# liruiluo/VLA-Adapter

Hardware: AMD Instinct MI355X
Metric: fine-tune samples/sec (224px img + 32-tok prompt), adapter-only, fwd+bwd+AdamW (higher is better)
Workload: dtype bf16

## Files before the change

include/vla_native.h:

```cpp
#ifndef VLA_NATIVE_H
#define VLA_NATIVE_H
#ifdef __cplusplus
extern "C" {
#endif

#define VLA_ERR_ARG (-1)
#define VLA_ERR_LAUNCH (-2)
#define VLA_ERR_UNSUPPORTED (-3)

#define VLA_ABI_VERSION 8
int vla_version(void);
int vla_desc_size(int which);
const char* vla_last_error(void);

enum { VLA_ACT_NONE = 0, VLA_ACT_GELU = 1, VLA_ACT_RELU = 2, VLA_ACT_GELU_TANH = 3, VLA_ACT_SWIGLU = 4, VLA_ACT_SWIGLU_BWD = 5 };

typedef struct vla_gemm_desc {
  const void* A;
  const void* B;
  void* C;
  const void* bias;
  const void* R;
  void* C2;
  int M, N, K, lda, ldb, ldc, ldr, ldc2;
// ... 49 lines not shown
int vla_layernorm_fwd_q8(void* stream, const void* x, const void* w, const void* b, void* y, float* stats, void* q8, float* qscale, int rows,
                         int cols, int ldx, int ldy, int ldq, float eps);

int vla_gemm_bf16_nt(void* stream, const vla_gemm_desc* desc );

int vla_transpose_bf16(void* stream, const void* in, void* out, int rows, int cols, int ldi, int ldo, int batch,
                       long long s_in, long long s_out);

int vla_layernorm_fwd(void* stream, const void* x, const void* w, const void* b, void* y, float* stats, int rows,
                      int cols, int ldx, int ldy, float eps);
int vla_layernorm_bwd(void* stream, const void* dy, const void* x, const void* w, const float* stats, void* dx,
                      float* dw, float* db, int rows, int cols, int ldx, int lddy, int lddx);
int vla_rmsnorm_fwd(void* stream, const void* x, const void* w, void* y, float* rstd, int rows, int cols, float eps);
int vla_rmsnorm_bwd(void* stream, const void* dy, const void* x, const void* w, const float* rstd, const void* dres,
                    void* dx, int rows, int cols, int x_group, int x_group_rows, int x_row0);

int vla_rmsnorm_dw(void* stream, const void* dy, const void* x, const float* rstd, float* dw, int rows, int cols);

typedef struct vla_attn_desc {
  const void* q; const void* k; const void* v;
  void* o;
  float* lse;
  const unsigned char* kmask;
  long long q_sb, k_sb, v_sb, o_sb;
  int q_ss, k_ss, v_ss, o_ss;
  int B, Sq, Sk, Hq, Hkv, dh, causal;
  float scale;
  const void* dout; void* dq; void* dk; void* dv; float* delta;
  long long do_sb, dq_sb, dk_sb, dv_sb; int do_ss, dq_ss, dk_ss, dv_ss;
  const float* rope_cos; const float* rope_sin;
// ... 117 lines not shown
```

vla_adapter_amd/csrc/gemm.hip:

```cpp
#include <algorithm>
#include "common.h"
#include "gemm_params.h"
#include "../../include/vla_native.h"

namespace {

constexpr int BK = 64;
constexpr int EPI_PAD = 16;


__device__ __forceinline__ float apply_act(float v, int act) {
  switch (act) {
    case VLA_ACT_GELU: return rbf(gelu_erf(v));
    case VLA_ACT_RELU: return fmaxf(v, 0.f);
    case VLA_ACT_GELU_TANH: return rbf(gelu_tanh(v));
    default: return v;
  }
}

typedef int v8i_f8 __attribute__((ext_vector_type(8)));
__device__ __forceinline__ v8i_f8 cat8(bf16x8 lo, bf16x8 hi) {
  typedef float f32x8 __attribute__((ext_vector_type(8)));
  const f32x4 l = __builtin_bit_cast(f32x4, lo), h = __builtin_bit_cast(f32x4, hi);
  return __builtin_bit_cast(v8i_f8, f32x8{l[0], l[1], l[2], l[3], h[0], h[1], h[2], h[3]});
// ... 668 lines not shown
  if (d->fp8)
    VLA_REQUIRE(d->fp8 == 1 && d->a_scale && d->b_scale && d->K % 128 == 0 && d->lda % 16 == 0 && d->ldb % 16 == 0 && d->batch == 1 &&
                    d->split_k <= 1 && d->rope_mode != 2 && d->a_group == 0 && (d->act != VLA_ACT_SWIGLU_BWD || d->K2 > 0),
                "gemm: fp8 needs scales, K % 128 == 0, 16-B rows, batch 1, no split-K / interleaved RoPE / row groups on A (SwiGLU backward: with a K extension only)");
  VLA_REQUIRE(((uintptr_t)d->A & 15) == 0 && ((uintptr_t)d->B & 15) == 0, "gemm: A/B must be 16-B aligned");
  VLA_REQUIRE(d->sA % 8 == 0 && d->sB % 8 == 0, "gemm: batch strides of A/B must keep 16-B alignment");
  if (d->act == VLA_ACT_SWIGLU_BWD) {
    VLA_REQUIRE(d->C && d->R && !d->bias && d->rope_mode == 0 && d->N % 64 == 0 && d->ldc % 8 == 0 && d->ldr % 4 == 0 &&
                    ((uintptr_t)d->R & 7) == 0 && d->c_group == 0 && d->res_mod == 0,
                "gemm: swiglu_bwd needs C = dGU [M, 2N] (ldc%8), R = GU [M, 2N] (interleaved), N%64 == 0");
  } else if (d->act == VLA_ACT_SWIGLU) {
    VLA_REQUIRE(d->C2 && d->N % 32 == 0 && d->ldc2 % 4 == 0 && ((uintptr_t)d->C2 & 7) == 0 && d->sC2 % 4 == 0,
                "gemm: swiglu needs C2, N%32==0, ldc2%4==0");
    VLA_REQUIRE(!d->R, "gemm: swiglu epilogue takes no residual");
  } else {
    VLA_REQUIRE(d->C, "gemm: null C");
  }
  if (d->C) VLA_REQUIRE(((uintptr_t)d->C & 15) == 0 || (d->ldc % 8) != 0, "gemm: C must be 16-B aligned");
  if (d->C && d->ldc % 8 == 0) VLA_REQUIRE(d->sC % 8 == 0, "gemm: sC must keep 16-B alignment");
  if (d->R && d->ldc % 8 == 0 && d->ldr % 8 == 0 && d->act != VLA_ACT_SWIGLU_BWD)
    VLA_REQUIRE(((uintptr_t)d->R & 15) == 0 && d->sR % 8 == 0, "gemm: R must be 16-B aligned");
  VLA_REQUIRE(d->a_group >= 0 && d->c_group >= 0 && d->a_group_stride % 8 == 0 &&
                  (d->c_group == 0 || d->ldc % 8 != 0 || d->c_group_stride % 8 == 0),
              "gemm: row-group strides must keep 16-B alignment");
  const bool split_k = d->split_k > 1;
  VLA_REQUIRE(d->bias_post_round == 0 || (d->bias_post_round == 1 && d->bias && d->rope_mode != 1 && !split_k && d->act == VLA_ACT_NONE),
              "gemm: bias_post_round needs a bias and a plain epilogue (no rotate_half rope / split-K / activation)");
  if (split_k) {
    VLA_REQUIRE(d->ws && d->batch == 1 && d->rope_mode == 0 && d->c_group == 0 && d->r_group == 0 &&
                    d->res_mod == 0 && d->c_live_mod == 0 && d->C &&
                    (d->act == VLA_ACT_NONE || d->act == VLA_ACT_GELU || d->act == VLA_ACT_RELU || d->act == VLA_ACT_GELU_TANH),
                "gemm: split_k needs an fp32 workspace [split_k, M, N], batch 1 and a plain epilogue");
    VLA_REQUIRE(d->N % 4 == 0 && ((uintptr_t)d->ws & 15) == 0, "gemm: split_k needs N % 4 == 0 and a 16-B aligned workspace");
  }
  VLA_REQUIRE(d->c_live_mod >= 0 && d->c_live_from >= 0 && (d->c_live_mod == 0 || d->c_live_from < d->c_live_mod),
              "gemm: c_live_from must lie inside c_live_mod");
  VLA_REQUIRE(d->r_group >= 0 && d->r_group_stride % 8 == 0 && (d->r_group == 0 || d->res_mod == 0),
              "gemm: r_group stride must keep 16-B alignment; r_group and res_mod are exclusive");
  if (d->K2 != 0)
    VLA_REQUIRE(d->K2 > 0 && d->K2 % BK == 0 && d->A2 && d->B2 && d->lda2 % 8 == 0 && d->ldb2 % 8 == 0 && (((uintptr_t)d->A2 | (uintptr_t)d->B2) & 15) == 0 &&
                    d->batch == 1 && !split_k && d->rope_mode != 2,
                "gemm: the K extension needs A2 / B2 (bf16, 16-B aligned rows, K2 % 64 == 0), batch 1, no split-K / interleaved RoPE");
  if (d->rope_mode != 0) {
    VLA_REQUIRE(d->rope_mode == 1 || d->rope_mode == 2, "gemm: rope_mode 0/1/2");
    VLA_REQUIRE(d->rope_cos && d->rope_sin && d->rope_T > 0 && d->rope_dh > 0 && d->rope_dh % 4 == 0 && d->rope_cols % 64 == 0 &&
                    (((uintptr_t)d->rope_cos | (uintptr_t)d->rope_sin) & 15) == 0 && d->act != VLA_ACT_SWIGLU,
                "gemm: bad rope arguments");
// ... 39 lines not shown
  else if (pl.kernel == VLA_KERNEL_NT_256)
    rc = vla_gemm256_launch(p, d->act == VLA_ACT_SWIGLU ? 1 : d->act == VLA_ACT_SWIGLU_BWD ? 2 : 0, d->batch, ov.grid_set ? ov.grid : ncu, st);
  else if (d->K2 > 0 && d->fp8)
    rc = rope == 3 ? launch_nt<3, true, true>(pl.kernel, p, nb, st) : rope == 1 ? launch_nt<1, true, true>(pl.kernel, p, nb, st)
                                                                                : launch_nt<0, true, true>(pl.kernel, p, nb, st);
  else if (d->K2 > 0)
    rc = rope == 3 ? launch_nt<3, false, true>(pl.kernel, p, nb, st) : rope == 1 ? launch_nt<1, false, true>(pl.kernel, p, nb, st)
                                                                                 : launch_nt<0, false, true>(pl.kernel, p, nb, st);
  else if (d->fp8) rc = rope == 1 ? launch_nt<1, true>(pl.kernel, p, nb, st) : launch_nt<0, true>(pl.kernel, p, nb, st);
  else if (rope == 3) rc = launch_nt<3>(pl.kernel, p, nb, st);
  else if (rope == 2) rc = launch_nt<2>(pl.kernel, p, nb, st);
  else if (rope == 1) rc = launch_nt<1>(pl.kernel, p, nb, st);
  else rc = launch_nt<0>(pl.kernel, p, nb, st);
  if (rc) return rc;
  VLA_CHECK_LAUNCH("gemm_bf16_nt");
  if (pl.split > 1) return splitk_finalize(d, pl.split, st);
  return VLA_OK;
}
```

vla_adapter_amd/csrc/norm.hip:

```cpp
#include "common.h"
#include "../../include/vla_native.h"

namespace {

template <int NCH>
__device__ __forceinline__ void load_row(const bf16_t* x, int cols, int lane, uint4 (&v)[NCH]) {
#pragma unroll
  for (int c = 0; c < NCH; ++c) {
    const int e = (c * 64 + lane) * 8;
    v[c] = (e < cols) ? *reinterpret_cast<const uint4*>(x + e) : uint4{0, 0, 0, 0};
  }
}
__device__ __forceinline__ void unpack8(const uint4& u, float (&f)[8]) {
  const unsigned w[4] = {u.x, u.y, u.z, u.w};
#pragma unroll
  for (int k = 0; k < 4; ++k) {
    f[2 * k] = __uint_as_float(w[k] << 16);
    f[2 * k + 1] = __uint_as_float(w[k] & 0xffff0000u);
  }
}
__device__ __forceinline__ uint4 pack8(const float (&f)[8]) {
  return uint4{pack2(f[0], f[1]), pack2(f[2], f[3]), pack2(f[4], f[5]), pack2(f[6], f[7])};
}

// ... 193 lines not shown
  for (int c = 0; c < NCH; ++c) {
    const int e = (c * 64 + lane) * 8;
    if (e >= cols) continue;
    float f[8], fw[8], o[8];
    unpack8(v[c], f);
    unpack8(vw[c], fw);
#pragma unroll
    for (int k = 0; k < 8; ++k) o[k] = fw[k] * rbf(f[k] * rstd);
    v[c] = pack8(o);
    if (y) *reinterpret_cast<uint4*>(y + (long long)row * cols + e) = v[c];
  }
  if (q8) quant_row_q8<NCH>(v, cols, lane, q8 + (long long)row * ldq, qscale + row);
}

template <int NCH>
__global__ __launch_bounds__(256) void rmsnorm_bwd_kernel(const bf16_t* __restrict__ dy, const bf16_t* __restrict__ x,
                                                          const bf16_t* __restrict__ w, const float* __restrict__ rstd_in,
                                                          const bf16_t* __restrict__ dres, bf16_t* __restrict__ dx,
                                                          int rows, int cols, int xg, int xgr, int xr0) {
  const int lane = threadIdx.x & 63;
  const int row = blockIdx.x * 4 + (threadIdx.x >> 6);
  if (row >= rows) return;
  const long long xrow = xg > 0 ? (long long)(row / xg) * xgr + xr0 + (row % xg) : row;
  uint4 vx[NCH], vd[NCH], vw[NCH], vr[NCH];
  load_row<NCH>(x + xrow * cols, cols, lane, vx);
  load_row<NCH>(dy + (long long)row * cols, cols, lane, vd);
  load_row<NCH>(w, cols, lane, vw);
  if (dres) load_row<NCH>(dres + (long long)row * cols, cols, lane, vr);
  const float rstd = rstd_in[xrow];
  float s = 0.f;
#pragma unroll
  for (int c = 0; c < NCH; ++c) {
    const int e = (c * 64 + lane) * 8;
    if (e >= cols) continue;
    float fx[8], fd[8], fw[8];
    unpack8(vx[c], fx);
    unpack8(vd[c], fd);
    unpack8(vw[c], fw);
#pragma unroll
    for (int k = 0; k < 8; ++k) s += fd[k] * fw[k] * fx[k] * rstd;
  }
  s = wave_sum(s) / cols;
#pragma unroll
  for (int c = 0; c < NCH; ++c) {
    const int e = (c * 64 + lane) * 8;
    if (e >= cols) continue;
    float fx[8], fd[8], fw[8], o[8];
    unpack8(vx[c], fx);
    unpack8(vd[c], fd);
    unpack8(vw[c], fw);
    float fr[8] = {0, 0, 0, 0, 0, 0, 0, 0};
    if (dres) unpack8(vr[c], fr);
#pragma unroll
    for (int k = 0; k < 8; ++k) o[k] = fr[k] + rstd * (fd[k] * fw[k] - fx[k] * rstd * s);
    *reinterpret_cast<uint4*>(dx + (long long)row * cols + e) = pack8(o);
  }
}

inline int nch_for(int cols) { return (cols + 511) / 512; }

#define DISPATCH_NCH(n, CALL)                    \
  if (n <= 1) { CALL(1); }                       \
  else if (n <= 2) { CALL(2); }                  \
  else if (n <= 3) { CALL(3); }                  \
  else if (n <= 4) { CALL(4); }                  \
  else if (n <= 8) { CALL(8); }                  \
  else if (n <= 16) { CALL(16); }                \
  else { CALL(24); }

// ... 72 lines not shown
extern "C" int vla_rmsnorm_fwd_q8(void* stream, const void* x, const void* w, void* y, float* rstd, void* q8, float* qscale, int rows, int cols,
                                  int ldq, float eps) {
  VLA_REQUIRE(x && w && q8 && qscale && rows > 0 && cols > 0, "rmsnorm_fwd_q8: null/empty");
  VLA_REQUIRE(cols % 8 == 0 && cols <= 12288 && ldq % 16 == 0 && ldq >= cols, "rmsnorm_fwd_q8: cols%8==0, cols<=12288, ldq%16");
  VLA_REQUIRE((((uintptr_t)x | (uintptr_t)y | (uintptr_t)w | (uintptr_t)q8) & 15) == 0, "rmsnorm_fwd_q8: 16-B alignment");
  const int n = nch_for(cols);
  dim3 grid((rows + 3) / 4);
#define CALL(N) hipLaunchKernelGGL(rmsnorm_fwd_kernel<N>, grid, dim3(256), 0, (hipStream_t)stream, (const bf16_t*)x, (const bf16_t*)w, (bf16_t*)y, \
                                   rstd, rows, cols, eps, (unsigned char*)q8, qscale, ldq)
  DISPATCH_NCH(n, CALL)
#undef CALL
  VLA_CHECK_LAUNCH("rmsnorm_fwd_q8");
  return VLA_OK;
}

extern "C" int vla_rmsnorm_bwd(void* stream, const void* dy, const void* x, const void* w, const float* rstd,
                               const void* dres, void* dx, int rows, int cols, int x_group, int x_group_rows, int x_row0) {
  VLA_REQUIRE(dy && x && w && rstd && dx && rows > 0 && cols > 0, "rmsnorm_bwd: null/empty");
  VLA_REQUIRE(x_group >= 0 && (x_group == 0 || (x_row0 >= 0 && x_row0 + x_group <= x_group_rows)), "rmsnorm_bwd: bad row window");
  VLA_REQUIRE(cols % 8 == 0 && cols <= 12288, "rmsnorm_bwd: cols%8==0");
  const int n = nch_for(cols);
  dim3 grid((rows + 3) / 4);
#define CALL(N) hipLaunchKernelGGL(rmsnorm_bwd_kernel<N>, grid, dim3(256), 0, (hipStream_t)stream, (const bf16_t*)dy, \
                                   (const bf16_t*)x, (const bf16_t*)w, rstd, (const bf16_t*)dres, (bf16_t*)dx, rows, cols, \
                                   x_group, x_group_rows, x_row0)
  DISPATCH_NCH(n, CALL)
#undef CALL
  VLA_CHECK_LAUNCH("rmsnorm_bwd");
  return VLA_OK;
}


template <int LPR>
__global__ __launch_bounds__(CR_THREADS) void rmsnorm_dw_kernel(const bf16_t* __restrict__ dy, const bf16_t* __restrict__ x,
                                                                const float* __restrict__ rstd, float* __restrict__ dw, int rows, int cols) {
  __shared__ float sm[CR_THREADS / 64][64];
  const int c = CR<LPR>::col();
  float a[8] = {0, 0, 0, 0, 0, 0, 0, 0};
  if (c < cols)
    for (int r = CR<LPR>::row0(); r < rows; r += CR<LPR>::GROUPS) {
      float fd[8], fx[8];
      unpack8(*reinterpret_cast<const uint4*>(dy + (long long)r * cols + c), fd);
      unpack8(*reinterpret_cast<const uint4*>(x + (long long)r * cols + c), fx);
#pragma unroll
// ... 25 lines not shown
```

vla_adapter_amd/engine.py:

```python
from __future__ import annotations

import math
import os
from dataclasses import dataclass, field
from typing import Dict, List, Optional, Tuple

import torch

from . import ops, schedule
from .ops import ACT_GELU, ACT_GELU_TANH, ACT_NONE, ACT_RELU, ACT_SWIGLU, BF16
from .schedule import Segment, capture_graph, chunks, turnaround_chunks

NUM_TOKENS = 64
IGNORE_INDEX = -100


def rup(n: int, m: int) -> int:
    return (n + m - 1) // m * m


def copy_flat(dst: torch.Tensor, src: torch.Tensor):
    n = src.numel()
    ops.copy2d(src, dst, 1, n, n, n)

# ... 155 lines not shown
        q, s_ = self._qscratch(x.shape[0], x.shape[1], "n")
        ops.rmsnorm_fwd_q8(x, w, eps, q, s_, rstd=rstd, y=out if self.keep_norm_out else None)
        return self._hand_over(out, q, s_)

    def _lin(self, key, x, W, bias=None, **kw):
        wq = self.Q.get(key)
        if wq is not None:
            xq, xs = self._quant(x, "f")
            return ops.gemm_nt(xq, wq[0], bias=bias, fp8=(xs, wq[1]), **kw)
        return ops.gemm_nt(x, W, bias=bias, **kw)

    def _lin_bwd(self, key, dy, x, WT, out=None, swiglu_gu=None, **kw):
        if swiglu_gu is not None:
            return ops.gemm_swiglu_bwd(dy, WT, swiglu_gu, out=out, **kw)
        return ops.gemm_nt(dy, WT, out=out)


class ViT:

    def __init__(self, cfg: ViTCfg, sd: Dict[str, torch.Tensor], device, j: int = 0):
        self.cfg, self.key = cfg, f"vit{j}."
        self.lin = Linear(device)
        d, P = cfg.d, cfg.patch
        g = lambda k: sd[k].to(device=device, dtype=BF16).contiguous()
        self.kpe = rup(3 * P * P, 64)
        wpe = torch.zeros(d, self.kpe, device=device, dtype=BF16)
        wpe[:, :3 * P * P] = g("patch_embed.proj.weight").reshape(d, -1)
        self.wpe, self.bpe = wpe, g("patch_embed.proj.bias")
        self.pos = g("pos_embed").reshape(-1, d)
        assert self.pos.shape[0] == cfg.n_patches, "pos_embed covers patches only (no_embed_class / no cls token)"
# ... 194 lines not shown

    def fwd_final(self):
        n, D = self.cfg.n_layers, self.cfg.d
        ops.rmsnorm_fwd(self.HS[n + 1].view(-1, D), self.norm, self.cfg.eps, out=self.HS[n].view(-1, D), rstd=self.RF)

    def enable_fp8(self):
        for i, L in enumerate(self.layers):
            self.lin.Q[f"llm.{i}.qkv"] = ops.quant_fp8_rows(L["wqkv"])
            self.lin.Q[f"llm.{i}.gu"] = ops.quant_fp8_rows(L["wgu"])
        self.lin.fp8 = True

    def backward(self, dHS: torch.Tensor, B: int, S: int, row0: int = 0, n_run: Optional[int] = None) -> torch.Tensor:
        n_run = self.cfg.n_layers if n_run is None else n_run
        self.bwd_begin(dHS, row0, n_run)
        for i in range(n_run - 1, -1, -1):
            self.bwd_layer(i, dHS)
        return self.bwd_result()

    def bwd_begin(self, dHS: torch.Tensor, row0: Optional[int] = 0, n_run: Optional[int] = None, lin: Optional[Linear] = None):
        n, S, D = self.cfg.n_layers, self.S, self.cfg.d
        self._n_run = n if n_run is None else n_run
        self._blin = lin = self.lin if lin is None else lin
        if row0 is None:
            self.r0, self.Rl, self._win = 0, S, None
        else:
            assert 0 <= row0 < S and row0 % 32 == 0, "live-row window must start on a multiple of 32"
            assert row0 >= self.gu_row0, "the forward dropped backward-only rows this window needs"
            self.r0, self.Rl = row0, S - row0
            self._win = (self.Rl, S, row0)
        Mr = self.B * self.Rl
        assert tuple(dHS.shape[1:]) == (self.B, self.Rl, D)
        d = (self.G_res[self._n_run - 1] if self.per_layer else self.d_a)[:Mr]
        if self._n_run == n:
            self._d = ops.rmsnorm_bwd(dHS[n].view(Mr, D), self.HS[n + 1].view(-1, D), self.norm, self.RF, out=d, x_rows=self._win)
            if lin.trains_vectors:
                ops.rmsnorm_dw(dHS[n].view(Mr, D), self.HS[n + 1].view(-1, D), self.RF, lin.A("llm.norm"))
        else:
            self._d = ops.copy2d(dHS[self._n_run].view(Mr, D), d, Mr, D, D, D)

    def bwd_layer(self, i: int, dHS: torch.Tensor):
        c, B, S, r0, R, lin = self.cfg, self.B, self.S, self.r0, self.Rl, self._blin
        M, D, H, KV, dh, I = B * S, c.d, c.heads, c.kv_heads, c.dh, c.inter
        Mr, tv, win = B * R, lin.trains_vectors, self._win
        L, k, d = self.layers[i], f"llm.{i}.", self._d
        _, n2, h = self._keeps(i)
        if self.per_layer:
            d1_out, d_out = self.G_d1[i], (self.G_res[i - 1] if i > 0 else self.d_last)[:Mr]
            d_gu, d_qkv = self.G_gu[i][:Mr], self.G_qkv[i][:Mr]
        else:
            d1_out, d_out, d_gu, d_qkv = self.d_b[:Mr], d, self.d_gu[:Mr], self.d_qkv[:Mr]
        if i < self._n_run - 1:
            ops.add_(d, dHS[i + 1].view(Mr, D))
        tap = lin.taps.get(("llm", i)) if lin.taps is not None else None
        if tap is not None:
            tap["d_out"] = d.clone()
        d_gu = lin._lin_bwd(k + "down", d, h, L["wdT"], out=d_gu, swiglu_gu=self.GU[i][r0:], **({"gu_group": (R, S * 2 * I)} if win else {}))
        d_n = lin._lin_bwd(k + "gu", d_gu, n2, L["wguT"], out=self.G_n2[i] if tv else self.d_n[:Mr])
        if tv:
            lin._defer(lambda dy=d_n, x=self.X1[i], r=self.R2[i], acc=lin.A(k + "n2"): ops.rmsnorm_dw(dy, x, r, acc))
        d1 = ops.rmsnorm_bwd(d_n, self.X1[i], L["n2"], self.R2[i], dres=d, out=d1_out, x_rows=win)
        dao = lin._lin_bwd(k + "o", d1, self.AO[i], L["woT"], out=self.d_n[:Mr])
        q, kk, v = self._attn_views(self.QKV[i].view(B, S, -1))
        dq, dk, dv = self._attn_views(d_qkv.view(B, R, -1))
        ops.attn_bwd(dao.view(B, R, -1), q[:, r0:], kk, v, self.AO[i].view(B, S, -1)[:, r0:], self.LSE[i], H, KV, dh, True,
                     self.kmask, dq=dq, dk=dk, dv=dv, rope=(self.cos, self.sin) if dh in (64, 128) else None, row0=r0)
        if dh not in (64, 128):
            cs, sn = self.cos[r0:], self.sin[r0:]
            ops.rope_half_(d_qkv[:, :H * dh], cs, sn, R, H, dh, sign=-1)
            ops.rope_half_(d_qkv[:, H * dh:(H + KV) * dh], cs, sn, R, KV, dh, sign=-1)
        d_n = lin._lin_bwd(k + "qkv", d_qkv, self._keeps(i)[0], L["wqkvT"], out=self.G_n1[i] if tv else self.d_n[:Mr])
        if tv:
            lin._defer(lambda dy=d_qkv, acc=lin.A(k + "bqkv"): ops.colsum_(dy, acc))
            lin._defer(lambda dy=d_n, x=self.HS[i].view(M, D), r=self.R1[i], acc=lin.A(k + "n1"): ops.rmsnorm_dw(dy, x, r, acc))
        self._d = ops.rmsnorm_bwd(d_n, self.HS[i].view(M, D), L["n1"], self.R1[i], dres=d1, out=d_out, x_rows=win)
        if tap is not None:
            tap["d_in"] = self._d.clone()

    def bwd_result(self) -> torch.Tensor:
        return self._d.view(self.B, self.Rl, self.cfg.d)


class FlatParams:

    def __init__(self, spec: List[Tuple[str, Tuple[int, ...]]], device):
        self.offsets, off = {}, 0
        for name, shape in spec:
            n = math.prod(shape)
            self.offsets[name] = (off, shape)
            off += rup(n, 8)
        self.numel = off
        self.data = torch.zeros(off, device=device, dtype=BF16)
        self.grad = torch.zeros(off, device=device, dtype=BF16)
        self.m = torch.zeros(off, device=device, dtype=BF16)
# ... 613 lines not shown
                self._prep_backward(batch)
                llm.fwd_begin(self.B, self.S, mm, self._row0_used)
            llm.fwd_layers(lo, hi)

        def turn_around():
            pred = head.fwd_end()
            self._loss3, dpred = ops.l1_loss(pred, self._actions_bf, True, 1.0 / self.ga)
            if self._guard is not None:
                ops.add_scalar_f32_(self._loss3, self._guard)
            head.bwd_begin(dpred, self._row0_used)

        def llm_bwd(k, lo, hi):
            if k == 0:
                llm.bwd_begin(self._dHS, self._row0_used, n)
            for i in range(hi - 1, lo - 1, -1):
                llm.bwd_layer(i, self._dHS)
            if k == len(fch) - 1:
                dq = ops.action_query_grad(llm.bwd_result().contiguous(), self.pos0, self.Np, self._row0_used)
                ops.cast_f32_bf16(dq, out=head.P.g("action_queries"))

        return (schedule.pipeline_forward(head, fch, llm_fwd, lambda: (llm.HS, self.pos1, batch["proprio"], self.Np, noise), turn_around,
                                          refresh=True)
                + schedule.pipeline_backward(head, fch, llm_bwd, lambda: self._dHS)
                + [Segment("H", head.bwd_end, None, ("end", 0))])

    def _stream_of(self, name: str, main):
        return main if name == "M" else self.side if name == "H" else self._vstreams[int(name[1:])]

    def _cap_stream(self, name: str):
        return self._cap_main if name == "M" else self._stream_of(name, None)

# ... 149 lines not shown
```

vla_adapter_amd/native.py:

```python
from __future__ import annotations

import ctypes as C
import os

_HERE = os.path.dirname(os.path.abspath(__file__))
LIB_PATH = (os.environ.get("VLA_NATIVE_LIB") or None) or os.path.join(_HERE, "libvla_native.so")

ACT_NONE, ACT_GELU, ACT_RELU, ACT_GELU_TANH, ACT_SWIGLU, ACT_SWIGLU_BWD = 0, 1, 2, 3, 4, 5
KERNEL_NT_SKINNY, KERNEL_NT_64x128_S6, KERNEL_NT_128x128_S4, KERNEL_NT_128x128, KERNEL_NT_128x64, KERNEL_NT_256 = 0, 8, 9, 10, 11, 12
KERNEL_TN_128, KERNEL_TN_256 = 16, 17
ABI_VERSION = 8


class NativeLibraryMissing(ImportError):
    pass


class GemmDesc(C.Structure):
    _fields_ = [("A", C.c_void_p), ("B", C.c_void_p), ("C", C.c_void_p), ("bias", C.c_void_p), ("R", C.c_void_p),
                ("C2", C.c_void_p),
                ("M", C.c_int), ("N", C.c_int), ("K", C.c_int), ("lda", C.c_int), ("ldb", C.c_int), ("ldc", C.c_int),
                ("ldr", C.c_int), ("ldc2", C.c_int), ("res_mod", C.c_int), ("act", C.c_int), ("batch", C.c_int),
                ("sA", C.c_longlong), ("sB", C.c_longlong), ("sC", C.c_longlong), ("sR", C.c_longlong),
                ("sC2", C.c_longlong), ("sBias", C.c_longlong), ("alpha", C.c_float),
# ... 49 lines not shown
    "vla_gemm256_extent_ok": ([C.POINTER(GemmDesc)], _I),
    "vla_gemm_nt_plan": ([C.POINTER(GemmDesc), _I, _I, C.POINTER(C.c_int)], _I),
    "vla_gemm_tn_plan": ([C.POINTER(GemmTnDesc), _I, C.POINTER(C.c_int)], _I),
    "vla_gemm_latency_hint": ([C.c_int], _I),
    "vla_gemm_bf16_tn": ([_P, C.POINTER(GemmTnDesc)], _I),
    "vla_gemm_bf16_tn_grouped": ([_P, C.POINTER(GemmTnDesc), _I], _I),
    "vla_copy_rows3d": ([_P, _P, _P, _I, _I, _I, _L, _L, _L, _L], _I),
    "vla_layerscale_fwd": ([_P, _P, _P, _P, _P, _L, _I], _I),
    "vla_layerscale_bwd": ([_P, _P, _P, _P, _P, _P, _I, _I], _I),
    "vla_gemm_bf16_nt": ([_P, C.POINTER(GemmDesc)], _I),
    "vla_transpose_bf16": ([_P, _P, _P, _I, _I, _I, _I, _I, _L, _L], _I),
    "vla_layernorm_fwd": ([_P, _P, _P, _P, _P, _P, _I, _I, _I, _I, _F], _I),
    "vla_layernorm_bwd": ([_P, _P, _P, _P, _P, _P, _P, _P, _I, _I, _I, _I, _I], _I),
    "vla_rmsnorm_fwd": ([_P, _P, _P, _P, _P, _I, _I, _F], _I),
    "vla_rmsnorm_bwd": ([_P, _P, _P, _P, _P, _P, _P, _I, _I, _I, _I, _I], _I),
    "vla_attn_fwd": ([_P, C.POINTER(AttnDesc)], _I),
    "vla_attn_bwd": ([_P, C.POINTER(AttnDesc)], _I),
    "vla_rope_half": ([_P, _P, _P, _P, _I, _I, _I, _I, _I, _I], _I),
    "vla_rope_interleaved": ([_P, _P, _P, _P, _I, _I, _I, _I, _I, _I], _I),
    "vla_im2col_patch": ([_P, _P, _P, _I, _I, _I, _I, _I, _I, _I, _I], _I),
    "vla_image_normalize_u8": ([_P, _P, _P, _I, _I, _I, _I, _I, C.POINTER(C.c_float), C.POINTER(C.c_float), _I], _I),
    "vla_action_tokenize": ([_P, _P, _P, _P, _L, _I, _F, _F, _L], _I),
    "vla_action_mask": ([_P, _P, _P, _P, _P, _I, _I, _I], _I),
    "vla_embed_splice": ([_P, _P, _P, _P, _P, _P, _P, _P, _I, _I, _I, _I, _I], _I),
    "vla_action_query_grad": ([_P, _P, _P, _P, _I, _I, _I, _I, _I], _I),
    "vla_gather_rows": ([_P, _P, _P, _P, _I, _I, _I, _I], _I),
    "vla_scatter_add_rows": ([_P, _P, _P, _P, _I, _I, _I, _I], _I),
    "vla_add_bf16": ([_P, _P, _P, _P, _L], _I),
    "vla_gelu_fwd": ([_P, _P, _P, _L], _I),
    "vla_gelu_bwd": ([_P, _P, _P, _P, _L], _I),
# ... 66 lines not shown
```

vla_adapter_amd/ops.py:

```python
from __future__ import annotations

import ctypes as C
import math
from typing import Optional, Tuple

import torch

from . import native as N
from .native import ACT_GELU, ACT_GELU_TANH, ACT_NONE, ACT_RELU, ACT_SWIGLU, ACT_SWIGLU_BWD

BF16 = torch.bfloat16


def _lib():
    return N.load()


def _st():
    return C.c_void_p(torch.cuda.current_stream().cuda_stream)


def _p(t: Optional[torch.Tensor]):
    return None if t is None else C.c_void_p(t.data_ptr())


def _chk_bf16(*ts):
    for t in ts:
        if t is not None:
            assert t.is_cuda and t.dtype == BF16, f"expected CUDA bf16 tensor, got {t.device} {t.dtype}"


def gemm_nt(a: torch.Tensor, b: torch.Tensor, *, bias=None, residual=None, res_mod: int = 0, act: int = ACT_NONE,
            out: Optional[torch.Tensor] = None, out2: Optional[torch.Tensor] = None, alpha: float = 1.0,
            want_pre: bool = True, a_group=None, c_group=None, r_group=None, rope=None, c_live=None,
            split_k: Optional[int] = None, bias_post_round: bool = False, fp8=None, ext=None, query_256: bool = False) -> torch.Tensor:
    if fp8 is not None:
        assert a.dtype == torch.uint8 and b.dtype == torch.uint8 and a.dim() == 2 and split_k in (None, 0, 1)
        _chk_bf16(bias, residual, out, out2)
        split_k = 0
    else:
        _chk_bf16(a, b, bias, residual, out, out2)
    assert a.stride(-1) == 1 and b.stride(-1) == 1
    batched = a.dim() == 3
    if batched:
        nb, M, K = a.shape
        sA = a.stride(0)
        sB = b.stride(0) if b.dim() == 3 else 0
        Nn = b.shape[-2]
    else:
        nb, (M, K), sA, sB, Nn = 1, a.shape, 0, 0, b.shape[0]
# ... 44 lines not shown
        assert sa.dtype == torch.float32 and sb.dtype == torch.float32 and sa.numel() == M and sb.numel() == Nn and sa.is_contiguous() and sb.is_contiguous()
        d.fp8, d.a_scale, d.b_scale = 1, sa.data_ptr(), sb.data_ptr()
    if ext is not None:
        a2, b2 = ext
        _chk_bf16(a2, b2)
        assert not batched and a2.dim() == 2 and b2.dim() == 2 and a2.shape[0] == M and b2.shape[0] == Nn and a2.shape[1] == b2.shape[1]
        assert a2.stride(1) == 1 and b2.stride(1) == 1 and a2.shape[1] % 64 == 0 and split_k in (None, 0, 1)
        d.A2, d.B2, d.K2, d.lda2, d.ldb2 = a2.data_ptr(), b2.data_ptr(), a2.shape[1], a2.stride(0), b2.stride(0)
        split_k = 0
    if bias_post_round:
        assert bias is not None
        d.bias_post_round = 1
    if split_k is None and not batched and K >= 2048:
        split_k = _nt_plan(d)[1]
    if split_k and split_k > 1:
        d.split_k, d.ws = split_k, _splitk_ws(split_k * M * Nn, a.device).data_ptr()
    if query_256:
        return _nt_plan(d)[0] == N.KERNEL_NT_256
    N.check(_lib().vla_gemm_bf16_nt(_st(), C.byref(d)), "gemm_bf16_nt")
    if act == ACT_SWIGLU:
        return out, out2
    return out


def _nt_plan(d) -> Tuple[int, int]:
    split = C.c_int(0)
    kernel = _lib().vla_gemm_nt_plan(C.byref(d), -1, 0, C.byref(split))
    N.check(min(kernel, 0), "gemm_nt_plan")
    return kernel, split.value


class latency_hint:

    def __enter__(self):
        self.prev = _lib().vla_gemm_latency_hint(1)
        return self

# ... 203 lines not shown
    assert x.is_contiguous() and q8.dtype == torch.uint8 and q8.stride(-1) == 1
    rows = x.numel() // cols
    N.check(_lib().vla_rmsnorm_fwd_q8(_st(), _p(x), _p(w), _p(y), _p(rstd), _p(q8), _p(qscale), rows, cols, q8.stride(-2), eps), "rmsnorm_fwd_q8")
    return q8, qscale


def layernorm_fwd_q8(x2, w, b, eps: float, q8: torch.Tensor, qscale: torch.Tensor, y: Optional[torch.Tensor] = None, stats=None):
    _chk_bf16(x2, w, b, y)
    rows, cols = x2.shape
    assert x2.stride(-1) == 1 and q8.dtype == torch.uint8 and q8.stride(-1) == 1
    N.check(_lib().vla_layernorm_fwd_q8(_st(), _p(x2), _p(w), _p(b), _p(y), _p(stats), _p(q8), _p(qscale), rows, cols, x2.stride(0),
                                        y.stride(0) if y is not None else 0, q8.stride(0), eps), "layernorm_fwd_q8")
    return q8, qscale


def rmsnorm_bwd(dy, x, w, rstd, dres=None, out=None, x_rows=None):
    _chk_bf16(dy, x, w, dres)
    cols = x.shape[-1]
    assert x.is_contiguous() and dy.is_contiguous()
    rows = dy.numel() // cols
    g, gr, r0 = x_rows if x_rows is not None else (0, 0, 0)
    if x_rows is None:
        assert x.numel() == dy.numel()
    else:
        assert rows % g == 0 and (rows // g) * gr * cols <= x.numel() and rstd.numel() * cols >= (rows // g) * gr * cols
    dx = torch.empty_like(dy) if out is None else out
    if dres is not None:
        assert dres.is_contiguous() and dres.numel() >= dy.numel()
    N.check(_lib().vla_rmsnorm_bwd(_st(), _p(dy), _p(x), _p(w), _p(rstd), _p(dres), _p(dx), rows, cols, g, gr, r0), "rmsnorm_bwd")
    return dx


def rmsnorm_dw(dy, x, rstd, acc_f32):
    rows, cols = dy.shape
    N.check(_lib().vla_rmsnorm_dw(_st(), _p(dy), _p(x), _p(rstd), _p(acc_f32), rows, cols), "rmsnorm_dw")
    return acc_f32


def _attn_desc(q, k, v, o, lse, kmask, causal, scale, Hq, Hkv, dh):
    d = N.AttnDesc()
    B, Sq, Sk = q.shape[0], q.shape[1], k.shape[1]
    d.q, d.k, d.v, d.o = q.data_ptr(), k.data_ptr(), v.data_ptr(), o.data_ptr()
    d.lse = lse.data_ptr() if lse is not None else None
# ... 363 lines not shown
```

Before: 1301.

## Fuse split-K reduction and residual head-add into RMSNorm backward

The gate-up backward GEMM can now skip its split-K finalize pass and leave raw fp32 partial planes. The RMSNorm backward kernel sums those planes directly. The RMSNorm backward also folds in the next layer's dHS gradient add, which removes a separate add_ kernel per layer. The last kernel of a chunk's layer is deferred so the fold can happen across chunk boundaries. This trades a finalize launch and a bf16 round trip for more fp32 reads inside the norm kernel, and changes rounding slightly.

```diff
diff --git a/include/vla_native.h b/include/vla_native.h
--- a/include/vla_native.h
+++ b/include/vla_native.h
@@ -87,6 +87,10 @@
 int vla_rmsnorm_fwd(void* stream, const void* x, const void* w, void* y, float* rstd, int rows, int cols, float eps);
 int vla_rmsnorm_bwd(void* stream, const void* dy, const void* x, const void* w, const float* rstd, const void* dres,
                     void* dx, int rows, int cols, int x_group, int x_group_rows, int x_row0);
+
+int vla_rmsnorm_bwd_fused(void* stream, const void* dy, const float* dy_planes, int planes, void* dy_out, const void* x, const void* w,
+                          const float* rstd, const void* dres, const void* add, void* dx, int rows, int cols, int x_group,
+                          int x_group_rows, int x_row0);
 
 int vla_rmsnorm_dw(void* stream, const void* dy, const void* x, const float* rstd, float* dw, int rows, int cols);
 
diff --git a/vla_adapter_amd/csrc/gemm.hip b/vla_adapter_amd/csrc/gemm.hip
--- a/vla_adapter_amd/csrc/gemm.hip
+++ b/vla_adapter_amd/csrc/gemm.hip
@@ -706,7 +706,7 @@
                 "gemm: swiglu needs C2, N%32==0, ldc2%4==0");
     VLA_REQUIRE(!d->R, "gemm: swiglu epilogue takes no residual");
   } else {
-    VLA_REQUIRE(d->C, "gemm: null C");
+    VLA_REQUIRE(d->C || d->split_k > 1, "gemm: null C");
   }
   if (d->C) VLA_REQUIRE(((uintptr_t)d->C & 15) == 0 || (d->ldc % 8) != 0, "gemm: C must be 16-B aligned");
   if (d->C && d->ldc % 8 == 0) VLA_REQUIRE(d->sC % 8 == 0, "gemm: sC must keep 16-B alignment");
@@ -720,9 +720,11 @@
               "gemm: bias_post_round needs a bias and a plain epilogue (no rotate_half rope / split-K / activation)");
   if (split_k) {
     VLA_REQUIRE(d->ws && d->batch == 1 && d->rope_mode == 0 && d->c_group == 0 && d->r_group == 0 &&
-                    d->res_mod == 0 && d->c_live_mod == 0 && d->C &&
+                    d->res_mod == 0 && d->c_live_mod == 0 &&
                     (d->act == VLA_ACT_NONE || d->act == VLA_ACT_GELU || d->act == VLA_ACT_RELU || d->act == VLA_ACT_GELU_TANH),
                 "gemm: split_k needs an fp32 workspace [split_k, M, N], batch 1 and a plain epilogue");
+    VLA_REQUIRE(d->C || (!d->bias && !d->R && d->act == VLA_ACT_NONE && (d->alpha == 0.f || d->alpha == 1.f) && d->K / BK >= d->split_k),
+                "gemm: split_k without C leaves the raw planes: no bias / residual / activation / alpha, and as many K-tiles as slices");
     VLA_REQUIRE(d->N % 4 == 0 && ((uintptr_t)d->ws & 15) == 0, "gemm: split_k needs N % 4 == 0 and a 16-B aligned workspace");
   }
   VLA_REQUIRE(d->c_live_mod >= 0 && d->c_live_from >= 0 && (d->c_live_mod == 0 || d->c_live_from < d->c_live_mod),
@@ -792,6 +794,6 @@
   else rc = launch_nt<0>(pl.kernel, p, nb, st);
   if (rc) return rc;
   VLA_CHECK_LAUNCH("gemm_bf16_nt");
-  if (pl.split > 1) return splitk_finalize(d, pl.split, st);
+  if (pl.split > 1 && d->C) return splitk_finalize(d, pl.split, st);
   return VLA_OK;
 }
diff --git a/vla_adapter_amd/csrc/norm.hip b/vla_adapter_amd/csrc/norm.hip
--- a/vla_adapter_amd/csrc/norm.hip
+++ b/vla_adapter_amd/csrc/norm.hip
@@ -231,31 +231,60 @@
 }
 
 template <int NCH>
-__global__ __launch_bounds__(256) void rmsnorm_bwd_kernel(const bf16_t* __restrict__ dy, const bf16_t* __restrict__ x,
+__device__ __forceinline__ void load_row_planes(const float* __restrict__ ws, long long plane, int split, int cols, int lane, uint4 (&v)[NCH]) {
+  typedef float f32x4 __attribute__((ext_vector_type(4)));
+#pragma unroll
+  for (int c = 0; c < NCH; ++c) {
+    const int e = (c * 64 + lane) * 8;
+    if (e >= cols) { v[c] = uint4{0, 0, 0, 0}; continue; }
+    f32x4 lo[8], hi[8];
+#pragma unroll
+    for (int z = 0; z < 8; ++z) {
+      lo[z] = z < split ? *reinterpret_cast<const f32x4*>(ws + z * plane + e) : f32x4{0.f, 0.f, 0.f, 0.f};
+      hi[z] = z < split ? *reinterpret_cast<const f32x4*>(ws + z * plane + e + 4) : f32x4{0.f, 0.f, 0.f, 0.f};
+    }
+    f32x4 a = lo[0], b = hi[0];
+#pragma unroll
+    for (int z = 1; z < 8; ++z) { a += lo[z]; b += hi[z]; }
+    for (int z = 8; z < split; ++z) {
+      a += *reinterpret_cast<const f32x4*>(ws + z * plane + e);
+      b += *reinterpret_cast<const f32x4*>(ws + z * plane + e + 4);
+    }
+    const float f[8] = {a[0] + 0.f, a[1] + 0.f, a[2] + 0.f, a[3] + 0.f, b[0] + 0.f, b[1] + 0.f, b[2] + 0.f, b[3] + 0.f};
+    v[c] = pack8(f);
+  }
+}
+
+template <int NCH, bool PLANES>
+__global__ __launch_bounds__(256) void rmsnorm_bwd_kernel(const bf16_t* __restrict__ dy, const float* __restrict__ ws, int split,
+                                                          bf16_t* __restrict__ dy_out, const bf16_t* __restrict__ x,
                                                           const bf16_t* __restrict__ w, const float* __restrict__ rstd_in,
-                                                          const bf16_t* __restrict__ dres, bf16_t* __restrict__ dx,
-                                                          int rows, int cols, int xg, int xgr, int xr0) {
+                                                          const bf16_t* __restrict__ dres, const bf16_t* __restrict__ add,
+                                                          bf16_t* __restrict__ dx, int rows, int cols, int xg, int xgr, int xr0) {
   const int lane = threadIdx.x & 63;
   const int row = blockIdx.x * 4 + (threadIdx.x >> 6);
   if (row >= rows) return;
   const long long xrow = xg > 0 ? (long long)(row / xg) * xgr + xr0 + (row % xg) : row;
-  uint4 vx[NCH], vd[NCH], vw[NCH], vr[NCH];
+  uint4 vx[NCH], vd[NCH], vw[NCH], vr[NCH], va[NCH];
   load_row<NCH>(x + xrow * cols, cols, lane, vx);
-  load_row<NCH>(dy + (long long)row * cols, cols, lane, vd);
+  if constexpr (PLANES) load_row_planes<NCH>(ws + (long long)row * cols, (long long)rows * cols, split, cols, lane, vd);
+  else load_row<NCH>(dy + (long long)row * cols, cols, lane, vd);
   load_row<NCH>(w, cols, lane, vw);
   if (dres) load_row<NCH>(dres + (long long)row * cols, cols, lane, vr);
+  if (add) load_row<NCH>(add + (long long)row * cols, cols, lane, va);
   const float rstd = rstd_in[xrow];
   float s = 0.f;
 #pragma unroll
   for (int c = 0; c < NCH; ++c) {
     const int e = (c * 64 + lane) * 8;
     if (e >= cols) continue;
+    if (PLANES && dy_out) *reinterpret_cast<uint4*>(dy_out + (long long)row * cols + e) = vd[c];
     float fx[8], fd[8], fw[8];
     unpack8(vx[c], fx);
     unpack8(vd[c], fd);
     unpack8(vw[c], fw);
 #pragma unroll
-    for (int k = 0; k < 8; ++k) s += fd[k] * fw[k] * fx[k] * rstd;
+    for (int k = 0; k < 8; ++k) s = __fadd_rn(s, __fmul_rn(__fmul_rn(__fmul_rn(fd[k], fw[k]), fx[k]), rstd));
   }
   s = wave_sum(s) / cols;
 #pragma unroll
@@ -269,7 +298,14 @@
     float fr[8] = {0, 0, 0, 0, 0, 0, 0, 0};
     if (dres) unpack8(vr[c], fr);
 #pragma unroll
-    for (int k = 0; k < 8; ++k) o[k] = fr[k] + rstd * (fd[k] * fw[k] - fx[k] * rstd * s);
+    for (int k = 0; k < 8; ++k)
+      o[k] = __fmaf_rn(rstd, __fmaf_rn(fd[k], fw[k], -__fmul_rn(__fmul_rn(fx[k], rstd), s)), fr[k]);
+    if (add) {
+      float fa[8];
+      unpack8(va[c], fa);
+#pragma unroll
+      for (int k = 0; k < 8; ++k) o[k] = __fadd_rn(rbf(o[k]), fa[k]);
+    }
     *reinterpret_cast<uint4*>(dx + (long long)row * cols + e) = pack8(o);
   }
 }
@@ -372,20 +408,35 @@
   return VLA_OK;
 }
 
+extern "C" int vla_rmsnorm_bwd_fused(void* stream, const void* dy, const float* dy_planes, int planes, void* dy_out, const void* x,
+                                     const void* w, const float* rstd, const void* dres, const void* add, void* dx, int rows, int cols,
+                                     int x_group, int x_group_rows, int x_row0) {
+  VLA_REQUIRE((dy != nullptr) != (dy_planes != nullptr) && x && w && rstd && dx && rows > 0 && cols > 0, "rmsnorm_bwd: null/empty, or not exactly one of dy / dy_planes");
+  VLA_REQUIRE(x_group >= 0 && (x_group == 0 || (x_row0 >= 0 && x_row0 + x_group <= x_group_rows)), "rmsnorm_bwd: bad row window");
+  VLA_REQUIRE(cols % 8 == 0 && cols <= 12288, "rmsnorm_bwd: cols%8==0");
+  VLA_REQUIRE(!dy_planes || (planes >= 2 && ((uintptr_t)dy_planes & 15) == 0), "rmsnorm_bwd: dy_planes needs >= 2 planes, 16-B aligned");
+  VLA_REQUIRE(dy_planes || !dy_out, "rmsnorm_bwd: dy_out goes with dy_planes");
+  const int n = nch_for(cols);
+  dim3 grid((rows + 3) / 4);
+#define CALL(N)                                                                                                              \
+  if (dy_planes)                                                                                                             \
+    hipLaunchKernelGGL((rmsnorm_bwd_kernel<N, true>), grid, dim3(256), 0, (hipStream_t)stream, (const bf16_t*)nullptr, dy_planes, \
+                       planes, (bf16_t*)dy_out, (const bf16_t*)x, (const bf16_t*)w, rstd, (const bf16_t*)dres, (const bf16_t*)add, \
+                       (bf16_t*)dx, rows, cols, x_group, x_group_rows, x_row0);                                              \
+  else                                                                                                                       \
+    hipLaunchKernelGGL((rmsnorm_bwd_kernel<N, false>), grid, dim3(256), 0, (hipStream_t)stream, (const bf16_t*)dy,           \
+                       (const float*)nullptr, 0, (bf16_t*)nullptr, (const bf16_t*)x, (const bf16_t*)w, rstd, (const bf16_t*)dres, \
+                       (const bf16_t*)add, (bf16_t*)dx, rows, cols, x_group, x_group_rows, x_row0)
+  DISPATCH_NCH(n, CALL)
+#undef CALL
+  VLA_CHECK_LAUNCH("rmsnorm_bwd");
+  return VLA_OK;
+}
+
 extern "C" int vla_rmsnorm_bwd(void* stream, const void* dy, const void* x, const void* w, const float* rstd,
                                const void* dres, void* dx, int rows, int cols, int x_group, int x_group_rows, int x_row0) {
-  VLA_REQUIRE(dy && x && w && rstd && dx && rows > 0 && cols > 0, "rmsnorm_bwd: null/empty");
-  VLA_REQUIRE(x_group >= 0 && (x_group == 0 || (x_row0 >= 0 && x_row0 + x_group <= x_group_rows)), "rmsnorm_bwd: bad row window");
-  VLA_REQUIRE(cols % 8 == 0 && cols <= 12288, "rmsnorm_bwd: cols%8==0");
-  const int n = nch_for(cols);
-  dim3 grid((rows + 3) / 4);
-#define CALL(N) hipLaunchKernelGGL(rmsnorm_bwd_kernel<N>, grid, dim3(256), 0, (hipStream_t)stream, (const bf16_t*)dy, \
-                                   (const bf16_t*)x, (const bf16_t*)w, rstd, (const bf16_t*)dres, (bf16_t*)dx, rows, cols, \
-                                   x_group, x_group_rows, x_row0)
-  DISPATCH_NCH(n, CALL)
-#undef CALL
-  VLA_CHECK_LAUNCH("rmsnorm_bwd");
-  return VLA_OK;
+  VLA_REQUIRE(dy, "rmsnorm_bwd: null/empty");
+  return vla_rmsnorm_bwd_fused(stream, dy, nullptr, 0, nullptr, x, w, rstd, dres, nullptr, dx, rows, cols, x_group, x_group_rows, x_row0);
 }
 
 
diff --git a/vla_adapter_amd/engine.py b/vla_adapter_amd/engine.py
--- a/vla_adapter_amd/engine.py
+++ b/vla_adapter_amd/engine.py
@@ -193,6 +193,11 @@
         if swiglu_gu is not None:
             return ops.gemm_swiglu_bwd(dy, WT, swiglu_gu, out=out, **kw)
         return ops.gemm_nt(dy, WT, out=out)
+
+    def _lin_bwd_planes(self, key, dy, x, WT, out):
+        if type(self)._lin_bwd is not Linear._lin_bwd:
+            return self._lin_bwd(key, dy, x, WT, out=out)
+        return ops.gemm_nt(dy, WT, out=out, planes=True)
 
 
 class ViT:
@@ -417,13 +422,14 @@
         n_run = self.cfg.n_layers if n_run is None else n_run
         self.bwd_begin(dHS, row0, n_run)
         for i in range(n_run - 1, -1, -1):
-            self.bwd_layer(i, dHS)
+            self.bwd_layer(i, dHS, fold_head=True)
         return self.bwd_result()
 
     def bwd_begin(self, dHS: torch.Tensor, row0: Optional[int] = 0, n_run: Optional[int] = None, lin: Optional[Linear] = None):
         n, S, D = self.cfg.n_layers, self.S, self.cfg.d
         self._n_run = n if n_run is None else n_run
         self._blin = lin = self.lin if lin is None else lin
+        self._tail, self._d_has_head = None, False
         if row0 is None:
             self.r0, self.Rl, self._win = 0, S, None
         else:
@@ -441,7 +447,9 @@
         else:
             self._d = ops.copy2d(dHS[self._n_run].view(Mr, D), d, Mr, D, D, D)
 
-    def bwd_layer(self, i: int, dHS: torch.Tensor):
+    def bwd_layer(self, i: int, dHS: torch.Tensor, fold_head: bool = False, defer_tail: bool = False):
+        if self._tail is not None:
+            self._tail()
         c, B, S, r0, R, lin = self.cfg, self.B, self.S, self.r0, self.Rl, self._blin
         M, D, H, KV, dh, I = B * S, c.d, c.heads, c.kv_heads, c.dh, c.inter
         Mr, tv, win = B * R, lin.trains_vectors, self._win
@@ -452,13 +460,14 @@
             d_gu, d_qkv = self.G_gu[i][:Mr], self.G_qkv[i][:Mr]
         else:
             d1_out, d_out, d_gu, d_qkv = self.d_b[:Mr], d, self.d_gu[:Mr], self.d_qkv[:Mr]
-        if i < self._n_run - 1:
+        if i < self._n_run - 1 and not self._d_has_head:
             ops.add_(d, dHS[i + 1].view(Mr, D))
         tap = lin.taps.get(("llm", i)) if lin.taps is not None else None
+        fold_head = fold_head and i > 0 and lin.taps is None
         if tap is not None:
             tap["d_out"] = d.clone()
         d_gu = lin._lin_bwd(k + "down", d, h, L["wdT"], out=d_gu, swiglu_gu=self.GU[i][r0:], **({"gu_group": (R, S * 2 * I)} if win else {}))
-        d_n = lin._lin_bwd(k + "gu", d_gu, n2, L["wguT"], out=self.G_n2[i] if tv else self.d_n[:Mr])
+        d_n = (lin._lin_bwd if tv else lin._lin_bwd_planes)(k + "gu", d_gu, n2, L["wguT"], out=self.G_n2[i] if tv else self.d_n[:Mr])
         if tv:
             lin._defer(lambda dy=d_n, x=self.X1[i], r=self.R2[i], acc=lin.A(k + "n2"): ops.rmsnorm_dw(dy, x, r, acc))
         d1 = ops.rmsnorm_bwd(d_n, self.X1[i], L["n2"], self.R2[i], dres=d, out=d1_out, x_rows=win)
@@ -475,11 +484,20 @@
         if tv:
             lin._defer(lambda dy=d_qkv, acc=lin.A(k + "bqkv"): ops.colsum_(dy, acc))
             lin._defer(lambda dy=d_n, x=self.HS[i].view(M, D), r=self.R1[i], acc=lin.A(k + "n1"): ops.rmsnorm_dw(dy, x, r, acc))
-        self._d = ops.rmsnorm_bwd(d_n, self.HS[i].view(M, D), L["n1"], self.R1[i], dres=d1, out=d_out, x_rows=win)
+        def tail():
+            self._tail, self._d_has_head = None, fold_head
+            self._d = ops.rmsnorm_bwd(d_n, self.HS[i].view(M, D), L["n1"], self.R1[i], dres=d1, out=d_out, x_rows=win,
+                                      add=dHS[i].view(Mr, D) if fold_head else None)
+        if defer_tail:
+            assert tap is None
+            self._tail = tail
+            return
+        tail()
         if tap is not None:
             tap["d_in"] = self._d.clone()
 
     def bwd_result(self) -> torch.Tensor:
+        assert self._tail is None, "a deferred last kernel of bwd_layer is still pending"
         return self._d.view(self.B, self.Rl, self.cfg.d)
 
 
@@ -1123,7 +1141,7 @@
             if k == 0:
                 llm.bwd_begin(self._dHS, self._row0_used, n)
             for i in range(hi - 1, lo - 1, -1):
-                llm.bwd_layer(i, self._dHS)
+                llm.bwd_layer(i, self._dHS, fold_head=True, defer_tail=i == lo and lo > 0)
             if k == len(fch) - 1:
                 dq = ops.action_query_grad(llm.bwd_result().contiguous(), self.pos0, self.Np, self._row0_used)
                 ops.cast_f32_bf16(dq, out=head.P.g("action_queries"))
diff --git a/vla_adapter_amd/native.py b/vla_adapter_amd/native.py
--- a/vla_adapter_amd/native.py
+++ b/vla_adapter_amd/native.py
@@ -87,6 +87,7 @@
     "vla_layernorm_bwd": ([_P, _P, _P, _P, _P, _P, _P, _P, _I, _I, _I, _I, _I], _I),
     "vla_rmsnorm_fwd": ([_P, _P, _P, _P, _P, _I, _I, _F], _I),
     "vla_rmsnorm_bwd": ([_P, _P, _P, _P, _P, _P, _P, _I, _I, _I, _I, _I], _I),
+    "vla_rmsnorm_bwd_fused": ([_P, _P, _P, _I, _P, _P, _P, _P, _P, _P, _P, _I, _I, _I, _I, _I], _I),
     "vla_attn_fwd": ([_P, C.POINTER(AttnDesc)], _I),
     "vla_attn_bwd": ([_P, C.POINTER(AttnDesc)], _I),
     "vla_rope_half": ([_P, _P, _P, _P, _I, _I, _I, _I, _I, _I], _I),
diff --git a/vla_adapter_amd/ops.py b/vla_adapter_amd/ops.py
--- a/vla_adapter_amd/ops.py
+++ b/vla_adapter_amd/ops.py
@@ -2,7 +2,7 @@
 
 import ctypes as C
 import math
-from typing import Optional, Tuple
+from typing import NamedTuple, Optional, Tuple
 
 import torch
 
@@ -33,7 +33,8 @@
 def gemm_nt(a: torch.Tensor, b: torch.Tensor, *, bias=None, residual=None, res_mod: int = 0, act: int = ACT_NONE,
             out: Optional[torch.Tensor] = None, out2: Optional[torch.Tensor] = None, alpha: float = 1.0,
             want_pre: bool = True, a_group=None, c_group=None, r_group=None, rope=None, c_live=None,
-            split_k: Optional[int] = None, bias_post_round: bool = False, fp8=None, ext=None, query_256: bool = False) -> torch.Tensor:
+            split_k: Optional[int] = None, bias_post_round: bool = False, fp8=None, ext=None, query_256: bool = False,
+            planes: bool = False) -> torch.Tensor:
     if fp8 is not None:
         assert a.dtype == torch.uint8 and b.dtype == torch.uint8 and a.dim() == 2 and split_k in (None, 0, 1)
         _chk_bf16(bias, residual, out, out2)
@@ -108,13 +109,26 @@
     if split_k is None and not batched and K >= 2048:
         split_k = _nt_plan(d)[1]
     if split_k and split_k > 1:
-        d.split_k, d.ws = split_k, _splitk_ws(split_k * M * Nn, a.device).data_ptr()
+        ws = _splitk_ws(split_k * M * Nn, a.device)
+        d.split_k, d.ws = split_k, ws.data_ptr()
     if query_256:
         return _nt_plan(d)[0] == N.KERNEL_NT_256
+    if planes and d.split_k > 1:
+        assert bias is None and residual is None and act == ACT_NONE and alpha == 1.0 and K // 64 >= split_k
+        d.C = None
+        N.check(_lib().vla_gemm_bf16_nt(_st(), C.byref(d)), "gemm_bf16_nt")
+        return SplitKPlanes(ws, _nt_plan(d)[1], M, Nn)
     N.check(_lib().vla_gemm_bf16_nt(_st(), C.byref(d)), "gemm_bf16_nt")
     if act == ACT_SWIGLU:
         return out, out2
     return out
+
+
+class SplitKPlanes(NamedTuple):
+    ws: torch.Tensor
+    n: int
+    rows: int
+    cols: int
 
 
 def _nt_plan(d) -> Tuple[int, int]:
@@ -348,9 +362,25 @@
     return q8, qscale
 
 
-def rmsnorm_bwd(dy, x, w, rstd, dres=None, out=None, x_rows=None):
-    _chk_bf16(dy, x, w, dres)
+def rmsnorm_bwd(dy, x, w, rstd, dres=None, out=None, x_rows=None, add=None, dy_out=None):
     cols = x.shape[-1]
+    if isinstance(dy, SplitKPlanes):
+        assert dy.cols == cols and dy.n >= 2 and dy.ws.dtype == torch.float32 and dy.ws.numel() >= dy.n * dy.rows * cols
+        _chk_bf16(x, w, dres, add, dy_out)
+        rows = dy.rows
+        assert out is not None and out.is_contiguous() and out.numel() == rows * cols
+        assert dy_out is None or (dy_out.is_contiguous() and dy_out.numel() == rows * cols)
+        assert x.is_contiguous() and (x_rows is not None or x.numel() == rows * cols)
+        g, gr, r0 = x_rows if x_rows is not None else (0, 0, 0)
+        if x_rows is not None:
+            assert rows % g == 0 and (rows // g) * gr * cols <= x.numel() and rstd.numel() * cols >= (rows // g) * gr * cols
+        for t in (dres, add):
+            assert t is None or (t.is_contiguous() and t.numel() >= rows * cols)
+        N.check(_lib().vla_rmsnorm_bwd_fused(_st(), None, _p(dy.ws), dy.n, _p(dy_out), _p(x), _p(w), _p(rstd), _p(dres), _p(add), _p(out),
+                                             rows, cols, g, gr, r0), "rmsnorm_bwd_fused")
+        return out
+    assert dy_out is None
+    _chk_bf16(dy, x, w, dres, add)
     assert x.is_contiguous() and dy.is_contiguous()
     rows = dy.numel() // cols
     g, gr, r0 = x_rows if x_rows is not None else (0, 0, 0)
@@ -359,8 +389,12 @@
     else:
         assert rows % g == 0 and (rows // g) * gr * cols <= x.numel() and rstd.numel() * cols >= (rows // g) * gr * cols
     dx = torch.empty_like(dy) if out is None else out
-    if dres is not None:
-        assert dres.is_contiguous() and dres.numel() >= dy.numel()
+    for t in (dres, add):
+        assert t is None or (t.is_contiguous() and t.numel() >= dy.numel())
+    if add is not None:
+        N.check(_lib().vla_rmsnorm_bwd_fused(_st(), _p(dy), None, 0, None, _p(x), _p(w), _p(rstd), _p(dres), _p(add), _p(dx), rows, cols,
+                                             g, gr, r0), "rmsnorm_bwd_fused")
+        return dx
     N.check(_lib().vla_rmsnorm_bwd(_st(), _p(dy), _p(x), _p(w), _p(rstd), _p(dres), _p(dx), rows, cols, g, gr, r0), "rmsnorm_bwd")
     return dx
 
```

New measurement: 1304, median of 6. No clear change (+0.2%).
